# ayumiymk/DiG

Measured on AMD Instinct MI355X. Metric: pretrain images/sec (32x128, 2-view, mask 0.7) ViT-S/4, higher is better.
Workload: dtype bf16

## Files before the change

cpu_abi/dig_cpu.cpp:

```cpp
#include <algorithm>
#include <cmath>
#include <cstdint>
#include <cstring>
#include <vector>

typedef void* hipStream_t;
#include "../include/dig_block_types.h"
enum { DIG_OK = 0, DIG_ERR_ARG = -1, DIG_ERR_ALIGN = -2, DIG_ERR_LAUNCH = -3, DIG_ERR_UNSUPPORTED = -4 };
typedef uint16_t bf16_t;

struct dig_dropout_t {
  unsigned k0, k1, thr;
  float scale;
  unsigned pk0, pk1, pthr;
  float pscale;
  int rows_per_sample;
};

namespace {

inline float bf2f(bf16_t h) {
  const uint32_t u = (uint32_t)h << 16;
  float f;
  std::memcpy(&f, &u, 4);
// ... 1009 lines not shown
  for (int k = 0; k < 4; ++k) accs4[k] = stats6[(k >> 1) * 3 + 1 + (k & 1)] * acc_scale;
  return DIG_OK;
}
int dig_step_meters(const float* loss, const float* contra, const float* pixel, const float* accs4, const int* counts, int n_counts,
                    const float* grad_norm, float* out10, hipStream_t) {
  if (!loss || !contra || !pixel || !accs4 || !counts || n_counts <= 0 || !out10) return DIG_ERR_ARG;
  int lo = counts[0], hi = counts[0];
  for (int i = 1; i < n_counts; ++i) { lo = std::min(lo, counts[i]); hi = std::max(hi, counts[i]); }
  out10[0] = loss[0]; out10[1] = contra[0]; out10[2] = pixel[0];
  for (int k = 0; k < 4; ++k) out10[3 + k] = accs4[k];
  out10[7] = (float)lo; out10[8] = (float)hi; out10[9] = grad_norm ? grad_norm[0] : NAN;
  return DIG_OK;
}
int dig_ce_rows(float* logits, int n, int m, int label_offset, float gscale, float* out3, hipStream_t) {
  if (!logits || !out3 || n <= 0 || m <= 0 || label_offset < 0 || label_offset + n > m) return DIG_ERR_ARG;
  for (int i = 0; i < n; ++i) {
    float* row = logits + (size_t)i * m;
    const int label = i + label_offset;
    float mx = -3.0e38f;
    for (int j = 0; j < m; ++j) mx = std::max(mx, row[j]);
    const float zl = row[label];
    float s = 0.f;
    int gt = 0;
    for (int j = 0; j < m; ++j) { s += std::exp(row[j] - mx); gt += row[j] > zl; }
    const float lse = mx + std::log(s);
    for (int j = 0; j < m; ++j) row[j] = gscale * (std::exp(row[j] - mx) / s - (j == label ? 1.f : 0.f));
    out3[0] += lse - zl;
    if (gt < 1) out3[1] += 1.f;
    if (gt < 5) out3[2] += 1.f;
  }
  return DIG_OK;
}

static int adamw_core(float* p, const float* g, float* m, float* v, bf16_t* shadow, long long n, const unsigned char* group, float lr0,
                      float wd0, float lr1, float wd1, float beta1, float beta2, float eps, float inv_bc1, float inv_sqrt_bc2,
                      float grad_scale, const float* finite_gate) {
  if (finite_gate && !std::isfinite(finite_gate[0])) return DIG_OK;
#pragma omp parallel for
  for (long long i = 0; i < n; ++i) {
    const int grp = group[i >> 8] & 0x7f;
    if (grp == 2) {
      if (shadow) shadow[i] = f2bf(p[i]);
      continue;
    }
    const float lr = grp ? lr1 : lr0, wd = grp ? wd1 : wd0;
    const float gk = g[i] * grad_scale;
    float P = p[i] * (1.0f - lr * wd);
    const float M = m[i] * beta1 + gk * (1.0f - beta1);
    const float V = v[i] * beta2 + gk * gk * (1.0f - beta2);
    P -= (lr * inv_bc1) * (M / (std::sqrt(V) * inv_sqrt_bc2 + eps));
    p[i] = P; m[i] = M; v[i] = V;
    if (shadow) shadow[i] = f2bf(P);
  }
  return DIG_OK;
}

int dig_adamw_bias_corrections(float beta1, float beta2, int step, float* out2) {
  if (!out2 || step < 1) return DIG_ERR_ARG;
  out2[0] = (float)(1.0 / (1.0 - std::pow((double)beta1, (double)step)));
  out2[1] = (float)(1.0 / std::sqrt(1.0 - std::pow((double)beta2, (double)step)));
  return DIG_OK;
}

struct AdamTrMat { long long off, dst_off; int rows, cols, tile0, pad; };

int dig_adamw_step_tr(float* p, const float* g, float* m, float* v, void* bf16_shadow, long long n, const unsigned char* group_flags, float lr0,
// ... 557 lines not shown
```

dig_amd/build.py:

```python
import os
import subprocess
import sys
from concurrent.futures import ThreadPoolExecutor

HERE = os.path.dirname(os.path.abspath(__file__))
CSRC = os.path.join(HERE, "csrc")
LIBDIR = os.path.join(HERE, "lib")
LIB = os.path.join(LIBDIR, "libdig_hip.so")
FLAGS = ["--offload-arch=gfx950", "-O3", "-std=c++17", "-fPIC", "-munsafe-fp-atomics", "-ffp-contract=fast",
         "-Wno-unused-result"]
FLAGS.append("-fno-slp-vectorize")
EXTRA_FLAGS = {"keyview.hip": ["-ffp-contract=off"], "abiaug.hip": ["-ffp-contract=off"]}


def sources():
    return sorted(f for f in os.listdir(CSRC) if f.endswith(".hip"))


def source_hash() -> str:
    import hashlib
    h = hashlib.sha256()
    files = sorted(os.path.join(CSRC, f) for f in os.listdir(CSRC) if f.endswith((".hip", ".h", ".inc")))
    inc = os.path.join(os.path.dirname(HERE), "include")
    files += sorted(os.path.join(inc, f) for f in os.listdir(inc) if f.endswith(".h"))
# ... 25 lines not shown
    for s in sources():
        src = os.path.join(CSRC, s)
        obj = os.path.join(objdir, s[:-4] + ".o")
        if force or _stale(obj, [src] + headers):
            jobs.append((src, obj))

    def cc(job):
        src, obj = job
        cmd = [hipcc] + FLAGS + EXTRA_FLAGS.get(os.path.basename(src), []) + ["-I", os.path.join(os.path.dirname(HERE), "include"), "-c", src, "-o", obj]
        r = subprocess.run(cmd, capture_output=True, text=True)
        if r.returncode != 0:
            raise RuntimeError(f"hipcc failed for {src}:\n{r.stderr}")
        if verbose:
            print("[dig_amd.build] compiled", os.path.basename(src), flush=True)

    with ThreadPoolExecutor(max_workers=min(8, max(1, len(jobs)))) as ex:
        list(ex.map(cc, jobs))
    objs = [os.path.join(objdir, s[:-4] + ".o") for s in sources()]
    if force or jobs or _stale(LIB, objs):
        r = subprocess.run([hipcc, "--offload-arch=gfx950", "-shared", "-fPIC", "-o", LIB] + objs,
                           capture_output=True, text=True)
        if r.returncode != 0:
            raise RuntimeError("link failed:\n" + r.stderr)
        if verbose:
            print("[dig_amd.build] linked", LIB, flush=True)
    return LIB


HOT_KERNELS = ("mlp_chain_kernel<1, true, false>", "mlp_chain_kernel<2, true, false>", "mlp_chain_kernel<0, true, false>",
               "wgrad_wide_kernel<3, 7>", "attn_block_kernel<true, 2>", "attn_block_kernel<false, 2>", "attn_bwd_kernel<false, 3, false>", "attn_bwd_kernel<false, 3, true>",
               "gemm_wide_kernel<false, true, 0, 4, 3, 2, 2, false, 64, 2, false>", "gemm_pwide_kernel<4, false, false>",
               "keyview_sample_kernel", "keyview_stage_a_kernel", "keyview_stage_b_kernel",
               "abiaug_sample_kernel", "abiaug_warp_kernel", "abiaug_det_kernel", "abiaug_tail_kernel",
               "lexicon_search_kernel")
LLVM_BIN = os.environ.get("DIG_LLVM_BIN", "/opt/rocm/lib/llvm/bin")


def kernel_resources():
    import re
    import tempfile
    rows = []
    objdir = os.path.join(LIBDIR, "obj")
    with tempfile.TemporaryDirectory() as tmp:
        for o in sorted(f for f in os.listdir(objdir) if f.endswith(".o")):
            fat, dev = os.path.join(tmp, o + ".fat"), os.path.join(tmp, o + ".co")
            r = subprocess.run([os.path.join(LLVM_BIN, "llvm-objcopy"), f"--dump-section=.hip_fatbin={fat}", os.path.join(objdir, o)], capture_output=True, text=True)
            if r.returncode != 0 or not os.path.exists(fat):
                continue
            subprocess.run([os.path.join(LLVM_BIN, "clang-offload-bundler"), "--unbundle", "--type=o", f"--input={fat}",
                            "--targets=hipv4-amdgcn-amd-amdhsa--gfx950", f"--output={dev}"], check=True, capture_output=True)
            notes = subprocess.run([os.path.join(LLVM_BIN, "llvm-readelf"), "--notes", dev], check=True, capture_output=True, text=True).stdout
            for blk in notes.split("- .agpr_count")[1:]:
                f = {k: re.search(rf"\.{k}:\s+(\S+)", blk) for k in ("name", "private_segment_fixed_size", "vgpr_count", "sgpr_count")}
                if not all(f.values()):
                    continue
                mangled = f["name"].group(1)
                try:
                    dm = subprocess.run(["c++filt", mangled], capture_output=True, text=True).stdout.strip() or mangled
                except OSError:
                    dm = mangled
                short = re.sub(r"^void ", "", dm).replace("(anonymous namespace)::", "")
                rows.append({"name": short, "object": o, "scratch": int(f["private_segment_fixed_size"].group(1)),
                             "vgpr": int(f["vgpr_count"].group(1)), "sgpr": int(f["sgpr_count"].group(1)),
                             "hot": any(short.startswith(h) for h in HOT_KERNELS)})
    return rows


# ... 12 lines not shown
```

dig_amd/csrc/loss.hip:

```cpp
#include "common.h"

namespace {

__global__ void l2norm_fwd_kernel(const float* __restrict__ x, float* __restrict__ y, float* __restrict__ inv_norm, int n, int C,
                                  float eps) {
  const int r = blockIdx.x * (blockDim.x >> 6) + (threadIdx.x >> 6);
  const int lane = threadIdx.x & 63;
  if (r >= n) return;
  float s = 0.f;
  for (int c = lane; c < C; c += 64) { const float v = x[(size_t)r * C + c]; s += v * v; }
  s = wave_sum(s);
  const float inv = 1.0f / fmaxf(sqrtf(s), eps);
  for (int c = lane; c < C; c += 64) y[(size_t)r * C + c] = x[(size_t)r * C + c] * inv;
  if (lane == 0) inv_norm[r] = inv;
}

__global__ void l2norm_bwd_kernel(const float* __restrict__ dy, const float* __restrict__ y, const float* __restrict__ inv_norm,
                                  float* __restrict__ dx, int n, int C) {
  const int r = blockIdx.x * (blockDim.x >> 6) + (threadIdx.x >> 6);
  const int lane = threadIdx.x & 63;
  if (r >= n) return;
  float s = 0.f;
  for (int c = lane; c < C; c += 64) s += y[(size_t)r * C + c] * dy[(size_t)r * C + c];
  s = wave_sum(s);
// ... 79 lines not shown
      atomicAdd(out, lse - zl);
      if (gt < 0.5f) atomicAdd(out + 1, 1.f);
      if (gt < 4.5f) atomicAdd(out + 2, 1.f);
    }
    return;
  }
  __shared__ float red2[256];
  const float mine[3] = {lse - zl, gt < 0.5f ? 1.f : 0.f, gt < 4.5f ? 1.f : 0.f};
  float tot[3];
  if (dig_grid_sum_last<3>(ws, mine, tot, red2)) { out[0] += tot[0]; out[1] += tot[1]; out[2] += tot[2]; }
}

__global__ void infonce_finish_kernel(const float* __restrict__ stats6, float loss_scale, float acc_scale, float* __restrict__ contra,
                                      float* __restrict__ accs4) {
  if (threadIdx.x == 0) contra[0] = (stats6[0] + stats6[3]) * loss_scale;
  if (threadIdx.x < 4) accs4[threadIdx.x] = stats6[(threadIdx.x >> 1) * 3 + 1 + (threadIdx.x & 1)] * acc_scale;
}

__global__ __launch_bounds__(64) void step_meters_kernel(const float* __restrict__ loss, const float* __restrict__ contra, const float* __restrict__ pixel,
                                                        const float* __restrict__ accs4, const int* __restrict__ counts, int n_counts,
                                                        const float* __restrict__ grad_norm, float* __restrict__ out10) {
  int lo = 0x7fffffff, hi = -0x7fffffff - 1;
  for (int i = threadIdx.x; i < n_counts; i += 64) { const int c = counts[i]; lo = min(lo, c); hi = max(hi, c); }
#pragma unroll
  for (int o = 32; o > 0; o >>= 1) { lo = min(lo, __shfl_xor(lo, o, 64)); hi = max(hi, __shfl_xor(hi, o, 64)); }
  if (threadIdx.x == 0) {
    out10[0] = loss[0]; out10[1] = contra[0]; out10[2] = pixel[0];
    out10[7] = (float)lo; out10[8] = (float)hi;
    out10[9] = grad_norm ? grad_norm[0] : __builtin_nanf("");
  }
  if (threadIdx.x < 4) out10[3 + threadIdx.x] = accs4[threadIdx.x];
}

}

extern "C" int dig_infonce_finish(const float* stats6, float loss_scale, float acc_scale, float* contra, float* accs4, hipStream_t stream) {
  if (!stats6 || !contra || !accs4) return DIG_ERR_ARG;
  hipLaunchKernelGGL(infonce_finish_kernel, dim3(1), dim3(64), 0, stream, stats6, loss_scale, acc_scale, contra, accs4);
  return dig_check_launch();
}

extern "C" int dig_step_meters(const float* loss, const float* contra, const float* pixel, const float* accs4, const int* counts, int n_counts,
                               const float* grad_norm, float* out10, hipStream_t stream) {
  if (!loss || !contra || !pixel || !accs4 || !counts || n_counts <= 0 || !out10) return DIG_ERR_ARG;
  hipLaunchKernelGGL(step_meters_kernel, dim3(1), dim3(64), 0, stream, loss, contra, pixel, accs4, counts, n_counts, grad_norm, out10);
  return dig_check_launch();
}

extern "C" int dig_l2norm_fwd(const float* x, float* y, float* inv_norm, int n, int C, float eps, hipStream_t stream) {
  if (!x || !y || !inv_norm || n <= 0 || C <= 0) return DIG_ERR_ARG;
  hipLaunchKernelGGL(l2norm_fwd_kernel, dim3((n + 3) / 4), dim3(256), 0, stream, x, y, inv_norm, n, C, eps);
  return dig_check_launch();
}

extern "C" int dig_l2norm_bwd(const float* dy, const float* y, const float* inv_norm, float* dx, int n, int C, hipStream_t stream) {
  if (!dy || !y || !inv_norm || !dx || n <= 0 || C <= 0) return DIG_ERR_ARG;
  hipLaunchKernelGGL(l2norm_bwd_kernel, dim3((n + 3) / 4), dim3(256), 0, stream, dy, y, inv_norm, dx, n, C);
  return dig_check_launch();
}

extern "C" int dig_sgemm(const float* A, const float* B, float* C, int I, int J, int R, int lda, int ldb, int ldc, int trans_b,
                         float alpha, int r_splits, hipStream_t stream) {
  if (!A || !B || !C || I <= 0 || J <= 0 || R <= 0 || r_splits < 1) return DIG_ERR_ARG;
  const int per = ((R + r_splits - 1) / r_splits + 63) / 64 * 64;
  if ((R + per - 1) / per != r_splits) return DIG_ERR_ARG;
  dim3 grid((J + 31) / 32, (I + 31) / 32, r_splits);
  if (trans_b)
    hipLaunchKernelGGL(sgemm_kernel<true>, grid, dim3(256), 0, stream, A, B, C, I, J, R, lda, ldb, ldc, alpha, per);
  else
    hipLaunchKernelGGL(sgemm_kernel<false>, grid, dim3(256), 0, stream, A, B, C, I, J, R, lda, ldb, ldc, alpha, per);
  return dig_check_launch();
}

extern "C" int dig_ce_rows_ws(float* logits, int n, int m, int label_offset, float gscale, float* out3, float* workspace, hipStream_t stream) {
  if (!logits || !out3 || n <= 0 || m <= 0 || label_offset < 0 || label_offset + n > m) return DIG_ERR_ARG;
  hipLaunchKernelGGL(ce_rows_kernel, dim3(n), dim3(256), 0, stream, logits, n, m, label_offset, gscale, out3, workspace);
  return dig_check_launch();
}
extern "C" int dig_ce_rows(float* logits, int n, int m, int label_offset, float gscale, float* out3, hipStream_t stream) {
  return dig_ce_rows_ws(logits, n, m, label_offset, gscale, out3, nullptr, stream);
}
```

dig_amd/engine_core.py:

```python
import ctypes
import functools
import itertools
import os
import weakref
from typing import Optional, Tuple

import torch

from . import block_calls as BC
from . import encoder_blocks as EB
from . import ops
from .arena import enc_block_views
from .parallel import LOCAL, LocalComm, bn_backward, bn_forward

BF16, F32 = torch.bfloat16, torch.float32
FWD_MODE = os.environ.get("DIG_FWD_MODE", "flip")
CHAIN_BWD_EVERY = max(1, int(os.environ.get("DIG_CHAIN_BWD_EVERY", "1")))
CHAIN_BWD_PHASE = int(os.environ.get("DIG_CHAIN_BWD_PHASE", "0"))
BATCH_REDUCE = os.environ.get("DIG_BATCH_REDUCE", "0") == "1"
FUSED_QV_BIAS_SUMS = os.environ.get("DIG_FUSED_QV_BIAS", "1") != "0"
WGRAD_GROUPING = os.environ.get("DIG_WGRAD_GROUPING", "block")
WGRAD_INLINE = os.environ.get("DIG_WGRAD_INLINE", "1") == "1"
WGRAD_DEFER = os.environ.get("DIG_WGRAD_DEFER", "auto").strip().lower()
if WGRAD_DEFER not in ("auto", "0", "1"):
# ... 337 lines not shown
            enc_m, ks = momentum_branch()
            del enc_m
            main.wait_stream(hi_st)
        else:
            side.wait_stream(main)
            with torch.cuda.stream(side):
                enc_m, ks = momentum_branch(heads=not dist_mode)
            enc, self.saved_enc = self.encoder_forward(ew_on, images, aug, mask_u8, True, path=self.path_on)
            self.enc = enc
            if not dist_mode:
                qs = online_heads(enc)
                main.wait_stream(side)
                if side is not main:
                    ks.record_stream(main)
                del enc_m
            else:
                main.wait_stream(side)
                enc_m.record_stream(main)
                if pp:
                    (masked2, self.saved_pix), (masked_m, _) = self.mlp_forward_pair(enc[:B * N], "pix_projector", "online", True,
                                                                                      enc_m[:B * N], "pix_projector_m", "momentum", False)
                else:
                    masked2, self.saved_pix, masked_m = enc[:B * N], None, enc_m[:B * N]
                pooled, self.saved_pnet = extract(masked2, enc, "patch_extractor", "online", True)
                pooled_m, _ = extract(masked_m, enc_m, "momentum_patch_extractor", "momentum", False)
                (qs, self.saved_proj), (ks, _) = self.mlp_forward_pair(pooled, "encoder_projection_layer", "online", True,
                                                                        pooled_m, "momentum_projection_layer", "momentum", False)
                qs, self.saved_pred = self.mlp_forward(qs, "predictor", "online", True)
                del enc_m, masked_m, pooled_m
        _mark("forward: both encoders + heads joined", dev)
        M._flat["bn_count"] += 1
        n = B * M.n_patch
        dim = M.moco_dim
        qf = torch.empty((2 * n, dim), device=dev, dtype=F32)
        kf = torch.empty((2 * n, dim), device=dev, dtype=F32)
        ops.cast_bf16_to_f32(qs, qf)
        ops.cast_bf16_to_f32(ks, kf)
        qn, self.q_inv = ops.l2norm_fwd(qf)
        kn, _ = ops.l2norm_fwd(kf)
        self.qn = qn
        if dist_mode:
            kall = comm.all_gather_cat(kn.view(1, 2, n, dim))
            k1_all = kall[:, 0].reshape(comm.world * n, dim).contiguous()
            k2_all = kall[:, 1].reshape(comm.world * n, dim).contiguous()
        else:
            k1_all, k2_all = kn[:n], kn[n:]
        mk = comm.world * n
        stats = torch.zeros((2, 3), device=dev, dtype=F32)
        self.dqn = torch.empty((2 * n, dim), device=dev, dtype=F32)
        gs = 2.0 * M.T / n
        for half, kk in ((0, k2_all), (1, k1_all)):
            logits = torch.empty((n, mk), device=dev, dtype=F32)
            ops.sgemm(qn[half * n:(half + 1) * n], kk, logits, n, mk, dim, False, 1.0 / M.T)
            ops.ce_rows(logits, n * comm.rank, gs, stats[half])
            ops.sgemm(logits, kk, self.dqn[half * n:(half + 1) * n], n, dim, mk, True, 1.0 / M.T)
        contra, accs = ops.infonce_finish(stats, 2.0 * M.T / n, 100.0 / n)
        if not M.use_pixel_target:
            vis_out = torch.empty((0, 0, M.dec_classes), device=dev, dtype=F32)
            self.mim_views = 0
        elif vis_out is None:
            vis_out, _ = decoder()
        _mark("forward: InfoNCE + SimMIM decoder done", dev)
        return contra, accs, vis_out

    def _decoder_forward(self, mask_u8, images, mim_views):
        M = self.m
        B, N, dev = images.shape[0], M.N, images.device
        per = M._mask_count(mask_u8, B)
        Mrows = mim_views * B * per
        Mp = (Mrows + 63) // 64 * 64
        idx, cnt = ops.mask_to_index(mask_u8[:mim_views * B], per)
        M._last_mask_counts, M._last_idx, M._last_images = cnt, idx[:B], images
        M._last_idx_views = [idx[:B]] + ([(idx[B:] - B * N).clamp_min_(0)] if mim_views == 2 else [])
        self.idx, self.Mrows, self.Mp, self.per, self.mim_views = idx, Mrows, Mp, per, mim_views
        w16, f32 = M._w("online"), M._f32
        gath = ops.gather_rows(self.enc, idx, Mrows, Mp)
        h0 = ops.linear_fwd(gath, w16["pix_decoder.0.weight"])
        h1 = ops.linear_fwd(h0, w16["pix_decoder.1.weight"])
        h2, mu, rs = ops.layernorm_fwd(h1, f32["pix_decoder.2.weight"], f32["pix_decoder.2.bias"], M.ln_eps, gelu=True)
        pred = torch.empty((Mp, 64), device=dev, dtype=F32)
        C = M.dec_classes
        ops.gemm(h2, w16["pix_decoder.4.weight"], Mp, C, M.dec_dim, out=pred, out_kind=ops.OUT_F32, bias=f32["pix_decoder.4.bias"], ldc=64)
        self.saved_dec = (gath, h0, h1, h2, mu, rs)
        return pred[:Mrows, :C].reshape(mim_views * B, per, C)

    def _forward_gen_only(self, ew_on, images, aug, mask_u8, mim_views, training, fresh):
        M = self.m
        dev = images.device
        views = mim_views
        self.gen_views = views
        self.wT = None
        if training and ((ops.mlp_chain_supported(M.D, M.F, views * self.B * M.N) and (ops.MLP_CHAIN_MASK & 4)) or
                         (ops.DGRAD_DIRECT and views * self.B * M.N >= 8192)):
            self.wT = self.mlp_weight_transposes(ew_on, fresh)
        enc_raw, self.saved_enc = self.encoder_forward(ew_on, images, aug, mask_u8, True, views=views, path=self.path_on)
        f32 = M._f32
        self.enc, mu, rs = ops.layernorm_fwd(enc_raw, f32["encoder.norm.weight"], f32["encoder.norm.bias"], M.ln_eps)
        self.saved_norm = (enc_raw, mu, rs)
        vis_out = self._decoder_forward(mask_u8, images, mim_views)
        return torch.zeros((), device=dev, dtype=F32), torch.zeros(4, device=dev, dtype=F32), vis_out

    def backward(self, g_contra, g_vis):
        M = self.m
        B, D, N, nw = self.B, M.D, M.N, M.num_windows
        dev = self.enc.device
        w16, f32, g32 = M._w("online"), M._f32, M._g32
        contrast = g_contra is not None and M.use_moco_target
        if g_vis is not None and not M.use_pixel_target:
            g_vis = None
        self._assign, M._grads_fresh = bool(getattr(M, "_grads_fresh", False)), False
        _mark("backward: start (loss, MSE, autograd entry done)", dev)
        views = 2 if (contrast or (g_vis is not None and self.mim_views == 2)) else 1
        d_enc = torch.empty_like(self.enc) if contrast else torch.zeros((views * B * N, D), device=dev, dtype=BF16)
        n = B * M.n_patch
        if contrast:
            dqn = self.dqn
            ops.scale_by_device_scalar(dqn, g_contra.reshape(1).float())
            dq = ops.l2norm_bwd(dqn, self.qn, self.q_inv)
            dq16 = torch.empty(dq.shape, device=dev, dtype=BF16)
            ops.cast_f32_to_bf16(dq, dq16)
            dproj = self.mlp_backward(dq16, "predictor", self.saved_pred)
            self._grad_ready(dev, "predictor")
            dpool = self.mlp_backward(dproj, "encoder_projection_layer", self.saved_proj)
            self._grad_ready(dev, "encoder_projection_layer")
            acc = False
            if M.patchnet == 'regular':
                from . import patchnet
                dpool, dfeat = patchnet.backward(self, dpool, "patch_extractor", self.saved_pnet, 2 * B)
                self._grad_ready(dev, "patch_extractor")
                d_enc, acc = dfeat, True
            if M.patchnet == 'conv':
                from . import convpatchnet
                d_enc = convpatchnet.backward(self, dpool, "patch_extractor", self.saved_pnet, 2 * B)
                self._grad_ready(dev, "patch_extractor")
                if M.has_pix_projector:
                    self.mlp_backward(d_enc[:B * N], "pix_projector", self.saved_pix, dx_out=d_enc[:B * N])
                    self._grad_ready(dev, "pix_projector")
            elif M.has_pix_projector:
                dmasked2 = d_enc[:B * N] if acc else torch.empty((B * N, D), device=dev, dtype=BF16)
                ops.window_pool_bwd(dpool[:n], dmasked2, B, M.gh, M.gw, nw, D, acc)
                ops.window_pool_bwd(dpool[n:], d_enc[B * N:], B, M.gh, M.gw, nw, D, acc)
                self.mlp_backward(dmasked2, "pix_projector", self.saved_pix, dx_out=d_enc[:B * N])
                self._grad_ready(dev, "pix_projector")
            else:
                ops.window_pool_bwd(dpool[:n], d_enc[:B * N], B, M.gh, M.gw, nw, D, acc)
                ops.window_pool_bwd(dpool[n:], d_enc[B * N:], B, M.gh, M.gw, nw, D, acc)
        elif M.use_moco_target:
            for name in (("predictor", "encoder_projection_layer") + (("patch_extractor",) if M.patchnet != 'no_patchtrans' else ())
                         + (("pix_projector",) if M.has_pix_projector else ())):
                self.comm.grad_ready(M, name)
        if g_vis is not None:
            gath, h0, h1, h2, mu, rs = self.saved_dec
            Mrows, Mp, C, Dd = self.Mrows, self.Mp, M.dec_classes, M.dec_dim
# ... 133 lines not shown
```

dig_amd/ops.py:

```python
import ctypes
import os
from collections import namedtuple

import torch

from . import _lib as L

cf = ctypes.c_float
cll = ctypes.c_longlong
BF16 = torch.bfloat16
F32 = torch.float32

OUT_BF16, OUT_F32, OUT_F32_PARTIAL = 0, 1, 2
GEMM_BK_FWD, GEMM_BK_BWD = 64, 32
_ws = {}


def _stream_id(dev):
    if L._raw_stream is not None and dev.index is not None:
        return L._raw_stream(dev.index)
    return torch.cuda.current_stream(dev).cuda_stream


def _workspace(dev, numel):
# ... 829 lines not shown
    L.call("dig_bn_update_running", L.ptr(sums), cf(n_total), cf(momentum), L.ptr(rm), L.ptr(rv), rm.numel(), L.stream())


def bn_bwd_stats(dy, x, mean, rstd, gamma, beta, relu, sums, dbeta=None, dgamma=None):
    ws = _workspace2(x.device, _bn_ws_floats(x.shape[0], x.shape[1]))
    L.call("dig_bn_bwd_stats_acc", L.ptr(dy), L.ptr(x), L.ptr(mean), L.ptr(rstd), L.ptr(gamma), L.ptr(beta), int(relu), L.ptr(sums),
           L.ptr(dbeta), L.ptr(dgamma), L.ptr(ws), x.shape[0], x.shape[1], L.stream())


def bn_bwd_apply(dy, x, mean, rstd, gamma, beta, relu, sums, n_total):
    dx = torch.empty_like(x)
    L.call("dig_bn_bwd_apply", L.ptr(dy), L.ptr(x), L.ptr(mean), L.ptr(rstd), L.ptr(gamma), L.ptr(beta), int(relu), L.ptr(sums),
           cf(n_total), L.ptr(dx), x.shape[0], x.shape[1], L.stream())
    return dx


def l2norm_fwd(x, eps=1e-12):
    y = torch.empty_like(x)
    inv = torch.empty(x.shape[0], device=x.device, dtype=F32)
    L.call("dig_l2norm_fwd", L.ptr(x), L.ptr(y), L.ptr(inv), x.shape[0], x.shape[1], cf(eps), L.stream())
    return y, inv


def l2norm_bwd(dy, y, inv):
    dx = torch.empty_like(y)
    L.call("dig_l2norm_bwd", L.ptr(dy), L.ptr(y), L.ptr(inv), L.ptr(dx), y.shape[0], y.shape[1], L.stream())
    return dx


SGEMM_SPLIT_SMALL = os.environ.get("DIG_SGEMM_SPLIT_SMALL", "1") != "0"
SGEMM_SPLIT_MIN_R = 256


def sgemm(A, B, C, I, J, R, trans_b, alpha):
    sp = 1
    if R >= 2048 and C.stride(0) == J:
        sp = R // 512
        while sp > 1 and R % (64 * sp):
            sp -= 1
    elif SGEMM_SPLIT_SMALL and R >= SGEMM_SPLIT_MIN_R and I * J <= (1 << 18) and C.stride(0) == J and R % 256 == 0:
        sp = R // 128
    if sp > 1:
        ws = _workspace(A.device, sp * I * J)
        L.call("dig_sgemm", L.ptr(A), L.ptr(B), L.ptr(ws), I, J, R, A.stride(0), B.stride(0), J, int(trans_b), cf(alpha), sp, L.stream())
        L.call("dig_reduce_partials", L.ptr(ws), sp, cll(I * J), L.ptr(C), 0, L.stream())
    else:
        L.call("dig_sgemm", L.ptr(A), L.ptr(B), L.ptr(C), I, J, R, A.stride(0), B.stride(0), C.stride(0), int(trans_b), cf(alpha), 1, L.stream())


def ce_rows(logits, label_offset, gscale, out3):
    n = logits.shape[0]
    L.call("dig_ce_rows_ws", L.ptr(logits), n, logits.shape[1], label_offset, cf(gscale), L.ptr(out3),
           L.ptr(_loss_workspace(logits.device, "ce", 1 + 3 * n)), L.stream())


def infonce_finish(stats, loss_scale, acc_scale):
    contra = torch.empty((), device=stats.device, dtype=F32)
    accs = torch.empty(4, device=stats.device, dtype=F32)
    L.call("dig_infonce_finish", L.ptr(stats), cf(loss_scale), cf(acc_scale), L.ptr(contra), L.ptr(accs), L.stream())
    return contra, accs


def step_meters(loss, contra, pixel, accs4, counts, grad_norm):
    out = torch.empty(10, device=loss.device, dtype=F32)
    L.call("dig_step_meters", L.ptr(loss), L.ptr(contra), L.ptr(pixel), L.ptr(accs4), L.ptr(counts), counts.numel(), L.ptr(grad_norm), L.ptr(out),
           L.stream())
    return out


def cast_f32_to_bf16(x, y, n=None):
    L.call("dig_cast_f32_to_bf16", L.ptr(x), L.ptr(y), cll(x.numel() if n is None else n), L.stream())


def cast_bf16_to_f32(x, y, n=None):
    L.call("dig_cast_bf16_to_f32", L.ptr(x), L.ptr(y), cll(x.numel() if n is None else n), L.stream())


def fill_f32(x, value=0.0):
    L.call("dig_fill_f32", L.ptr(x), cll(x.numel()), cf(value), L.stream())


def scale_f32(x, s):
    L.call("dig_scale_f32", L.ptr(x), cll(x.numel()), cf(s), L.stream())


def scale_by_device_scalar(x, scalar, extra=1.0):
    L.call("dig_scale_by_device_scalar", L.ptr(x), cll(x.numel()), L.ptr(scalar), cf(extra), L.stream())


def pad_cast_rows(src, dst, M, C):
    L.call("dig_pad_cast_rows", L.ptr(src), L.ptr(dst), M, C, dst.shape[0], dst.stride(0), L.stream())


def axpy_f32(y, x, a=1.0):
    L.call("dig_axpy_f32", L.ptr(y), L.ptr(x), cll(x.numel()), cf(a), L.stream())
# ... 36 lines not shown
```

include/dig_hip.h:

```cpp
#ifndef DIG_HIP_H
#define DIG_HIP_H

#ifdef __cplusplus
extern "C" {
#endif

#ifndef __HIP_PLATFORM_AMD__
typedef struct ihipStream_t* hipStream_t;
#endif

#include "dig_aug_types.h"

#define DIG_GEMM_TILE_DEFAULT 0
#define DIG_GEMM_TILE_128x128_K32 32
#define DIG_GEMM_TILE_128x128_K64 64
#define DIG_GEMM_TILE_256x256 244
#define DIG_GEMM_TILE_256x192 264
#define DIG_GEMM_TILE_64x128 212
#define DIG_GEMM_TILE_128x64 221
#define DIG_GEMM_TILE_256x256_PERSISTENT 544
#define DIG_GEMM_TILE_256x192_PERSISTENT 564
int dig_gemm_bf16(const void* A, const void* B, void* C, int I, int J, int R, int lda, int ldb, int ldc, int trans_a,
                  int trans_b, int out_kind, const float* bias, const void* resid, int ldr, void* pre_act, int ldp, float alpha,
                  int alpha_cols, int act, int splits, int a_rows, int b_rows, int bk, float* colsum_partials,
// ... 92 lines not shown
int dig_patch_embed_bwd(const void* dy, const float* img, const unsigned char* mask, float* dW, float* dbias, float* dmask_token,
                        int n_img, int gh, int gw, int D, hipStream_t stream);
int dig_patchify_bf16(const float* img, const unsigned char* mask, void* out, int n_img, int gh, int gw, hipStream_t stream);
int dig_colsum_masked(const void* x, const unsigned char* mask, float* out_unmasked, float* out_masked, float* workspace,
                      int rows, int C, hipStream_t stream);

int dig_window_pool_fwd(const void* x, void* out, int out_is_f32, int n_img, int gh, int gw, int nwin, int D, hipStream_t stream);
int dig_window_pool_bwd(const void* dpool, void* dx, int n_img, int gh, int gw, int nwin, int D, int accumulate, hipStream_t stream);

int dig_im2col3x3(const void* x, void* col, int n_img, int H, int W, int C, int ldc, hipStream_t stream);
int dig_conv3x3_weight_flip(const void* w, void* wt, int c_out, int c_in, hipStream_t stream);
int dig_maxpool2x2_fwd(const void* x, void* y, unsigned char* idx, int n_img, int H, int W, int C, hipStream_t stream);
int dig_maxpool2x2_bwd(const void* dy, const unsigned char* idx, void* dx, int n_img, int H, int W, int C, hipStream_t stream);

int dig_mask_views_u8(const void* mask, int elem_kind, int B, int V, int N, int keep_views, unsigned char* out, hipStream_t stream);
int dig_mask_to_index(const unsigned char* mask, int* idx, int* count, int B, int N, int max_per_sample, hipStream_t stream);
int dig_gather_rows(const void* src, const int* idx, void* dst, int M, int M_pad, int D, hipStream_t stream);
int dig_scatter_rows_add(const void* src, const int* idx, void* dst, int M, int D, hipStream_t stream);
int dig_mim_target(const float* img, const int* idx, float* target, int M, int gh, int gw, int normalize , hipStream_t stream);
int dig_mse_fwd_bwd(const float* pred, int ld_pred, const float* target, int M, int C, float gscale, float* loss, void* dpred,
                    int ld_dpred, hipStream_t stream);

int dig_l2norm_fwd(const float* x, float* y, float* inv_norm, int n, int C, float eps, hipStream_t stream);
int dig_l2norm_bwd(const float* dy, const float* y, const float* inv_norm, float* dx, int n, int C, hipStream_t stream);
int dig_sgemm(const float* A, const float* B, float* C, int I, int J, int R, int lda, int ldb, int ldc, int trans_b, float alpha,
              int r_splits , hipStream_t stream);
int dig_ce_rows(float* logits, int n, int m, int label_offset, float gscale, float* out3, hipStream_t stream);
int dig_mse_fwd_bwd_ws(const float* pred, int ld_pred, const float* target, int M, int C, float gscale, float* loss, void* dpred,
                       int ld_dpred, float* workspace, hipStream_t stream);
int dig_ce_rows_ws(float* logits, int n, int m, int label_offset, float gscale, float* out3, float* workspace, hipStream_t stream);
int dig_infonce_finish(const float* stats6, float loss_scale, float acc_scale, float* contra, float* accs4, hipStream_t stream);
int dig_step_meters(const float* loss, const float* contra, const float* pixel, const float* accs4, const int* counts, int n_counts,
                    const float* grad_norm, float* out10, hipStream_t stream);

int dig_adamw_step(float* p, const float* g, float* m, float* v, void* bf16_shadow, long long n, const unsigned char* group_flags,
                   float lr0, float wd0, float lr1, float wd1, float beta1, float beta2, float eps, int step, float grad_scale,
                   const float* finite_gate, hipStream_t stream);
int dig_adamw_step_tr(float* p, const float* g, float* m, float* v, void* bf16_shadow, long long n, const unsigned char* group_flags,
                      float lr0, float wd0, float lr1, float wd1, float beta1, float beta2, float eps, int step, float grad_scale,
                      const float* finite_gate, const void* mats, int n_mats, int n_tiles, void* tr_out, hipStream_t stream);
int dig_adamw_step_groups(float* p, const float* g, float* m, float* v, void* bf16_shadow, long long n, const unsigned char* group_idx,
                          const float* lr_tab, const float* wd_tab, float beta1, float beta2, float eps, int step, float grad_scale,
                          const float* finite_gate, hipStream_t stream);
int dig_ema_update(float* pm, const float* p, void* bf16_shadow, long long n, float m, hipStream_t stream);
int dig_adamw_bias_corrections(float beta1, float beta2, int step, float* out2_host);
int dig_adamw_step_dev(float* p, const float* g, float* m, float* v, void* bf16_shadow, long long n, const unsigned char* group_flags,
                       const float* scalars6, float beta1, float beta2, float eps, float grad_scale, const float* finite_gate,
                       hipStream_t stream);
int dig_ema_update_dev(float* pm, const float* p, void* bf16_shadow, long long n, const float* m_and_one_minus_m, hipStream_t stream);
long long dig_sumsq_workspace_bytes(long long n);
int dig_sumsq(const float* x, long long n, float* workspace, float* out, hipStream_t stream);

long long dig_colsum_workspace_bytes(int rows, int C);
int dig_colsum(const void* x, float* out, float* workspace, int rows, int C, int ld, hipStream_t stream);
int dig_colsum_partials(const float* partials, int n_parts, int C, float* out, hipStream_t stream);
#define DIG_COLSUM_MAX_SEGS 112
typedef struct dig_colsum_seg { const float* partials; float* out; long long stride; int n_parts; int C; } dig_colsum_seg_t;
int dig_colsum_partials_multi(const dig_colsum_seg_t* segs, int n_segs, hipStream_t stream);
int dig_gelu_bwd(const void* dact, const void* pre, void* dpre, long long n, hipStream_t stream);
int dig_add_bf16(const void* a, const void* b, void* out, long long n, hipStream_t stream);
int dig_cast_f32_to_bf16(const float* x, void* y, long long n, hipStream_t stream);
int dig_cast_bf16_to_f32(const void* x, float* y, long long n, hipStream_t stream);
int dig_pad_cast_rows(const float* src, void* dst, int M, int C, int M_pad, int ld, hipStream_t stream);
int dig_fill_f32(float* x, long long n, float value, hipStream_t stream);
int dig_scale_f32(float* x, long long n, float s, hipStream_t stream);
int dig_scale_by_device_scalar(float* x, long long n, const float* scalar, float extra, hipStream_t stream);
// ... 129 lines not shown
```

Before: 6788.

## Fuse InfoNCE normalize, logits, softmax-CE and dq backward into dedicated kernels

Replaces the multi-launch InfoNCE path (bf16 casts, l2norm, two sgemms per direction, ce_rows, finish, scale, l2norm backward, cast) with three kernels. One normalizes the keys and writes a transposed copy, one computes per-block-of-8-query logits, softmax cross-entropy, gradient and dq with a last-block reduction of the stats, and one fuses scaling, l2norm backward and the bf16 cast. The aim is to cut launch count and intermediate global traffic while keeping the same split-K summation order as the sgemm path. In exchange the path handles only limited key counts and dims, uses 1024-thread blocks with low grid parallelism, and is bypassed in distributed mode.

```diff
diff --git a/cpu_abi/dig_cpu.cpp b/cpu_abi/dig_cpu.cpp
--- a/cpu_abi/dig_cpu.cpp
+++ b/cpu_abi/dig_cpu.cpp
@@ -1065,6 +1065,62 @@
   return DIG_OK;
 }
 
+int dig_infonce_keys(const void* k, float* kn, float* knT, int rows, int C, int rows_per_part, float eps, hipStream_t st) {
+  if (!k || !kn || !knT || rows <= 0 || C <= 0 || rows_per_part <= 0 || rows % rows_per_part) return DIG_ERR_ARG;
+  std::vector<float> x((size_t)rows * C), inv(rows);
+  const bf16_t* kb = (const bf16_t*)k;
+  for (size_t e = 0; e < x.size(); ++e) x[e] = bf2f(kb[e]);
+  dig_l2norm_fwd(x.data(), kn, inv.data(), rows, C, eps, st);
+  for (int r = 0; r < rows; ++r)
+    for (int c = 0; c < C; ++c)
+      knT[((size_t)(r / rows_per_part) * C + c) * rows_per_part + r % rows_per_part] = kn[(size_t)r * C + c];
+  return DIG_OK;
+}
+
+static void nce_sliced_gemm(const float* A, const float* B, float* C, int I, int J, int R, bool trans_b, float alpha, int per) {
+  for (int i = 0; i < I; ++i)
+    for (int j = 0; j < J; ++j) {
+      float tot = 0.f;
+      for (int r0 = 0; r0 < R; r0 += per) {
+        float acc = 0.f;
+        for (int r = r0; r < std::min(R, r0 + per); ++r) acc += A[(size_t)i * R + r] * (trans_b ? B[(size_t)r * J + j] : B[(size_t)j * R + r]);
+        tot += alpha * acc;
+      }
+      C[(size_t)i * J + j] = tot;
+    }
+}
+
+int dig_infonce_rows(const void* q, const float* kn_a, const float* knT_a, const float* kn_b, const float* knT_b, int n, int m, int C,
+                     int label_offset, float alpha, float gscale, float eps, int per_l, int per_d, float loss_scale, float acc_scale,
+                     float* qn, float* q_inv, float* dqn, float* contra, float* accs4, float* workspace, hipStream_t st) {
+  if (!q || !kn_a || !knT_a || !kn_b || !knT_b || !qn || !q_inv || !dqn || !contra || !accs4 || !workspace || n <= 0 || m <= 0 || C <= 0 ||
+      label_offset < 0 || label_offset + n > m || per_l <= 0 || per_d <= 0)
+    return DIG_ERR_ARG;
+  if (m > 1024 || C > 256 || ((C + per_l - 1) / per_l) * (long long)m > 2048 || ((m + per_d - 1) / per_d) * (long long)C > 2048) return DIG_ERR_UNSUPPORTED;
+  std::vector<float> x((size_t)2 * n * C), logits((size_t)n * m);
+  const bf16_t* qb = (const bf16_t*)q;
+  for (size_t e = 0; e < x.size(); ++e) x[e] = bf2f(qb[e]);
+  dig_l2norm_fwd(x.data(), qn, q_inv, 2 * n, C, eps, st);
+  float stats[6] = {0.f, 0.f, 0.f, 0.f, 0.f, 0.f};
+  for (int dir = 0; dir < 2; ++dir) {
+    const float* kn = dir ? kn_b : kn_a;
+    nce_sliced_gemm(qn + (size_t)dir * n * C, kn, logits.data(), n, m, C, false, alpha, per_l);
+    dig_ce_rows(logits.data(), n, m, label_offset, gscale, stats + 3 * dir, st);
+    nce_sliced_gemm(logits.data(), kn, dqn + (size_t)dir * n * C, n, C, m, true, alpha, per_d);
+  }
+  return dig_infonce_finish(stats, loss_scale, acc_scale, contra, accs4, st);
+}
+
+int dig_infonce_dq(const float* dqn, const float* qn, const float* q_inv, const float* gscalar, void* dq, int n, int C, hipStream_t st) {
+  if (!dqn || !qn || !q_inv || !gscalar || !dq || n <= 0 || C <= 0) return DIG_ERR_ARG;
+  std::vector<float> dy((size_t)n * C), dx((size_t)n * C);
+  for (size_t e = 0; e < dy.size(); ++e) dy[e] = dqn[e] * gscalar[0];
+  dig_l2norm_bwd(dy.data(), qn, q_inv, dx.data(), n, C, st);
+  bf16_t* o = (bf16_t*)dq;
+  for (size_t e = 0; e < dx.size(); ++e) o[e] = f2bf(dx[e]);
+  return DIG_OK;
+}
+
 static int adamw_core(float* p, const float* g, float* m, float* v, bf16_t* shadow, long long n, const unsigned char* group, float lr0,
                       float wd0, float lr1, float wd1, float beta1, float beta2, float eps, float inv_bc1, float inv_sqrt_bc2,
                       float grad_scale, const float* finite_gate) {
diff --git a/dig_amd/build.py b/dig_amd/build.py
--- a/dig_amd/build.py
+++ b/dig_amd/build.py
@@ -81,7 +81,8 @@
                "gemm_wide_kernel<false, true, 0, 4, 3, 2, 2, false, 64, 2, false>", "gemm_pwide_kernel<4, false, false>",
                "keyview_sample_kernel", "keyview_stage_a_kernel", "keyview_stage_b_kernel",
                "abiaug_sample_kernel", "abiaug_warp_kernel", "abiaug_det_kernel", "abiaug_tail_kernel",
-               "lexicon_search_kernel")
+               "lexicon_search_kernel",
+               "infonce_keys_kernel", "infonce_rows_kernel", "infonce_dq_kernel")
 LLVM_BIN = os.environ.get("DIG_LLVM_BIN", "/opt/rocm/lib/llvm/bin")
 
 
diff --git a/dig_amd/csrc/loss.hip b/dig_amd/csrc/loss.hip
--- a/dig_amd/csrc/loss.hip
+++ b/dig_amd/csrc/loss.hip
@@ -135,6 +135,253 @@
   if (threadIdx.x < 4) out10[3 + threadIdx.x] = accs4[threadIdx.x];
 }
 
+constexpr int NCE_RB = 8;
+constexpr int NCE_KG = 4;
+constexpr int NCE_CMAX = 256;
+
+__device__ __forceinline__ float nce_rounded(float v) {
+  asm volatile("" : "+v"(v));
+  return v;
+}
+
+__global__ void infonce_keys_kernel(const bf16_t* __restrict__ k, float* __restrict__ kn, float* __restrict__ knT, int rows, int C,
+                                    int rows_per_part, float eps) {
+  const int r = blockIdx.x * (blockDim.x >> 6) + (threadIdx.x >> 6);
+  const int lane = threadIdx.x & 63;
+  if (r >= rows) return;
+  float s = 0.f;
+  for (int c = lane; c < C; c += 64) { const float v = bf2f(k[(size_t)r * C + c]); s += v * v; }
+  s = wave_sum(s);
+  const float inv = 1.0f / fmaxf(sqrtf(s), eps);
+  const int part = r / rows_per_part, rp = r - part * rows_per_part;
+  float* t = knT + (size_t)part * C * rows_per_part + rp;
+  for (int c = lane; c < C; c += 64) {
+    const float y = bf2f(k[(size_t)r * C + c]) * inv;
+    kn[(size_t)r * C + c] = y;
+    t[(size_t)c * rows_per_part] = y;
+  }
+}
+
+__device__ __forceinline__ void nce_slice(const float* __restrict__ g, size_t ld, const float (*lds)[NCE_RB], int r0, int r1, float (&acc)[NCE_RB]) {
+#pragma unroll
+  for (int ii = 0; ii < NCE_RB; ++ii) acc[ii] = 0.f;
+  for (int r = r0; r < r1; r += 16) {
+    float kv[16];
+#pragma unroll
+    for (int e = 0; e < 16; ++e) kv[e] = g[(size_t)min(r + e, r1 - 1) * ld];
+#pragma unroll
+    for (int e = 0; e < 16; ++e)
+      if (r + e < r1) {
+        const float4 a = *reinterpret_cast<const float4*>(&lds[r + e][0]), b = *reinterpret_cast<const float4*>(&lds[r + e][4]);
+        acc[0] = fmaf(a.x, kv[e], acc[0]); acc[1] = fmaf(a.y, kv[e], acc[1]); acc[2] = fmaf(a.z, kv[e], acc[2]); acc[3] = fmaf(a.w, kv[e], acc[3]);
+        acc[4] = fmaf(b.x, kv[e], acc[4]); acc[5] = fmaf(b.y, kv[e], acc[5]); acc[6] = fmaf(b.z, kv[e], acc[6]); acc[7] = fmaf(b.w, kv[e], acc[7]);
+      }
+  }
+}
+
+__global__ __launch_bounds__(1024) void infonce_rows_kernel(const bf16_t* __restrict__ q, const float* __restrict__ kn_a,
+                                                            const float* __restrict__ knT_a, const float* __restrict__ kn_b,
+                                                            const float* __restrict__ knT_b, int n, int m, int C, int label_offset,
+                                                            float alpha, float gscale, float eps, int per_l, int per_d, float loss_scale,
+                                                            float acc_scale, float* __restrict__ qn, float* __restrict__ q_inv,
+                                                            float* __restrict__ dqn, float* __restrict__ contra, float* __restrict__ accs4,
+                                                            float* __restrict__ ws) {
+  __shared__ __attribute__((aligned(16))) float Qs[NCE_CMAX][NCE_RB];
+  __shared__ __attribute__((aligned(16))) float Dl[NCE_KG * 256][NCE_RB];
+  __shared__ float red[3][NCE_RB][4];
+  __shared__ unsigned last_flag;
+  const int nb = (n + NCE_RB - 1) / NCE_RB;
+  const int dir = blockIdx.x / nb, i0 = (blockIdx.x - dir * nb) * NCE_RB;
+  const float* __restrict__ kn = dir ? kn_b : kn_a;
+  const float* __restrict__ knT = dir ? knT_b : knT_a;
+  const int t = threadIdx.x, lane = t & 63, w = t >> 6;
+
+  if (w < NCE_RB) {
+    const int ii = w;
+    if (i0 + ii < n) {
+      const size_t g = (size_t)(dir * n + i0 + ii) * C;
+      float s = 0.f;
+      for (int c = lane; c < C; c += 64) { const float v = bf2f(q[g + c]); s += v * v; }
+      s = wave_sum(s);
+      const float inv = 1.0f / fmaxf(sqrtf(s), eps);
+      for (int c = lane; c < C; c += 64) {
+        const float y = bf2f(q[g + c]) * inv;
+        qn[g + c] = y;
+        Qs[c][ii] = y;
+      }
+      if (lane == 0) q_inv[dir * n + i0 + ii] = inv;
+    } else {
+      for (int c = lane; c < C; c += 64) Qs[c][ii] = 0.f;
+    }
+  }
+  __syncthreads();
+
+  {
+    const int nsl = (C + per_l - 1) / per_l, items = nsl * m;
+    float part[2][NCE_RB];
+#pragma unroll
+    for (int k = 0; k < 2; ++k) {
+      const int wi = t + 1024 * k;
+      if (wi < items) {
+        const int sl = wi / m, j = wi - sl * m;
+        nce_slice(knT + j, (size_t)m, Qs, sl * per_l, min(C, (sl + 1) * per_l), part[k]);
+      }
+    }
+    for (int sl = 0; sl < nsl; ++sl) {
+#pragma unroll
+      for (int k = 0; k < 2; ++k) {
+        const int wi = t + 1024 * k;
+        if (wi < items && wi / m == sl) {
+          const int j = wi - sl * m;
+#pragma unroll
+          for (int ii = 0; ii < NCE_RB; ++ii) Dl[j][ii] = (sl ? Dl[j][ii] : 0.f) + nce_rounded(part[k][ii] * alpha);
+        }
+      }
+      __syncthreads();
+    }
+  }
+
+  float lse[NCE_RB], zl[NCE_RB], gts[NCE_RB];
+  float lg[NCE_KG][NCE_RB], mx[NCE_RB];
+  if (t < 256) {
+#pragma unroll
+    for (int ii = 0; ii < NCE_RB; ++ii) {
+      float v = -3.0e38f;
+#pragma unroll
+      for (int u = 0; u < NCE_KG; ++u) {
+        lg[u][ii] = (t + 256 * u < m) ? Dl[t + 256 * u][ii] : 0.f;
+        if (t + 256 * u < m) v = fmaxf(v, lg[u][ii]);
+      }
+      v = wave_max(v);
+      if (lane == 0) red[0][ii][w] = v;
+      zl[ii] = Dl[min(i0 + ii + label_offset, m - 1)][ii];
+    }
+  }
+  __syncthreads();
+  if (t < 256) {
+#pragma unroll
+    for (int ii = 0; ii < NCE_RB; ++ii) {
+      mx[ii] = fmaxf(fmaxf(red[0][ii][0], red[0][ii][1]), fmaxf(red[0][ii][2], red[0][ii][3]));
+      float s = 0.f, gt = 0.f;
+#pragma unroll
+      for (int u = 0; u < NCE_KG; ++u)
+        if (t + 256 * u < m) {
+          const float z = lg[u][ii];
+          s += __expf(z - mx[ii]);
+          gt += (z > zl[ii]) ? 1.f : 0.f;
+        }
+      s = wave_sum(s);
+      gt = wave_sum(gt);
+      if (lane == 0) { red[1][ii][w] = s; red[2][ii][w] = gt; }
+    }
+  }
+  __syncthreads();
+  if (t < 256) {
+#pragma unroll
+    for (int ii = 0; ii < NCE_RB; ++ii) {
+      const float s = red[1][ii][0] + red[1][ii][1] + red[1][ii][2] + red[1][ii][3];
+      gts[ii] = red[2][ii][0] + red[2][ii][1] + red[2][ii][2] + red[2][ii][3];
+      lse[ii] = mx[ii] + __logf(s);
+      const float inv = 1.0f / s;
+      const int label = i0 + ii + label_offset;
+#pragma unroll
+      for (int u = 0; u < NCE_KG; ++u) {
+        const int j = t + 256 * u;
+        if (j < m) {
+          const float p = __expf(lg[u][ii] - mx[ii]) * inv;
+          Dl[j][ii] = gscale * (p - (j == label ? 1.f : 0.f));
+        }
+      }
+    }
+  }
+  __syncthreads();
+
+  {
+    const int nsl = (m + per_d - 1) / per_d, items = nsl * C;
+    float part[2][NCE_RB];
+#pragma unroll
+    for (int k = 0; k < 2; ++k) {
+      const int wi = t + 1024 * k;
+      if (wi < items) {
+        const int sl = wi / C, c = wi - sl * C;
+        nce_slice(kn + c, (size_t)C, Dl, sl * per_d, min(m, (sl + 1) * per_d), part[k]);
+      }
+    }
+    for (int sl = 0; sl < nsl; ++sl) {
+#pragma unroll
+      for (int k = 0; k < 2; ++k) {
+        const int wi = t + 1024 * k;
+        if (wi < items && wi / C == sl) {
+          const int c = wi - sl * C;
+#pragma unroll
+          for (int ii = 0; ii < NCE_RB; ++ii) Qs[c][ii] = (sl ? Qs[c][ii] : 0.f) + nce_rounded(part[k][ii] * alpha);
+        }
+      }
+      __syncthreads();
+    }
+    for (int e = t; e < NCE_RB * C; e += 1024) {
+      const int ii = e / C, c = e - ii * C;
+      if (i0 + ii < n) dqn[(size_t)(dir * n + i0 + ii) * C + c] = Qs[c][ii];
+    }
+  }
+
+  if (t == 0) {
+#pragma unroll
+    for (int ii = 0; ii < NCE_RB; ++ii)
+      if (i0 + ii < n) {
+        float* o = ws + 1 + 3 * (size_t)(dir * n + i0 + ii);
+        o[0] = lse[ii] - zl[ii]; o[1] = gts[ii] < 0.5f ? 1.f : 0.f; o[2] = gts[ii] < 4.5f ? 1.f : 0.f;
+      }
+    __threadfence();
+    last_flag = (atomicAdd(reinterpret_cast<unsigned*>(ws), 1u) == gridDim.x - 1) ? 1u : 0u;
+  }
+  __syncthreads();
+  if (!last_flag) return;
+  __threadfence();
+  float* fold = &Dl[0][0];
+  if (t < 256) {
+    float a[6];
+#pragma unroll
+    for (int v = 0; v < 6; ++v) a[v] = 0.f;
+    for (int b = t; b < n; b += 256) {
+#pragma unroll
+      for (int v = 0; v < 6; ++v)
+        a[v] += __hip_atomic_load(ws + 1 + 3 * (size_t)((v / 3) * n + b) + (v % 3), __ATOMIC_RELAXED, __HIP_MEMORY_SCOPE_AGENT);
+    }
+#pragma unroll
+    for (int v = 0; v < 6; ++v) {
+      a[v] = wave_sum(a[v]);
+      if (lane == 0) fold[w * 6 + v] = a[v];
+    }
+  }
+  __syncthreads();
+  if (t != 0) return;
+  float st[6];
+#pragma unroll
+  for (int v = 0; v < 6; ++v) {
+    float x = 0.f;
+    for (int ww = 0; ww < 4; ++ww) x += fold[ww * 6 + v];
+    st[v] = 0.f + x;
+  }
+  contra[0] = (st[0] + st[3]) * loss_scale;
+  accs4[0] = st[1] * acc_scale; accs4[1] = st[2] * acc_scale; accs4[2] = st[4] * acc_scale; accs4[3] = st[5] * acc_scale;
+  reinterpret_cast<unsigned*>(ws)[0] = 0u;
+}
+
+__global__ void infonce_dq_kernel(const float* __restrict__ dqn, const float* __restrict__ y, const float* __restrict__ inv_norm,
+                                  const float* __restrict__ gscalar, bf16_t* __restrict__ dq, int n, int C) {
+  const int r = blockIdx.x * (blockDim.x >> 6) + (threadIdx.x >> 6);
+  const int lane = threadIdx.x & 63;
+  if (r >= n) return;
+  const float sc = gscalar[0] * 1.0f;
+  float s = 0.f;
+  for (int c = lane; c < C; c += 64) s += y[(size_t)r * C + c] * nce_rounded(dqn[(size_t)r * C + c] * sc);
+  s = wave_sum(s);
+  const float inv = inv_norm[r];
+  for (int c = lane; c < C; c += 64)
+    dq[(size_t)r * C + c] = f2bf((nce_rounded(dqn[(size_t)r * C + c] * sc) - y[(size_t)r * C + c] * s) * inv);
+}
+
 }
 
 extern "C" int dig_infonce_finish(const float* stats6, float loss_scale, float acc_scale, float* contra, float* accs4, hipStream_t stream) {
@@ -183,3 +430,31 @@
 extern "C" int dig_ce_rows(float* logits, int n, int m, int label_offset, float gscale, float* out3, hipStream_t stream) {
   return dig_ce_rows_ws(logits, n, m, label_offset, gscale, out3, nullptr, stream);
 }
+
+extern "C" int dig_infonce_keys(const void* k, float* kn, float* knT, int rows, int C, int rows_per_part, float eps, hipStream_t stream) {
+  if (!k || !kn || !knT || rows <= 0 || C <= 0 || rows_per_part <= 0 || rows % rows_per_part) return DIG_ERR_ARG;
+  hipLaunchKernelGGL(infonce_keys_kernel, dim3((rows + 3) / 4), dim3(256), 0, stream, (const bf16_t*)k, kn, knT, rows, C, rows_per_part, eps);
+  return dig_check_launch();
+}
+
+extern "C" int dig_infonce_rows(const void* q, const float* kn_a, const float* knT_a, const float* kn_b, const float* knT_b, int n, int m, int C,
+                                int label_offset, float alpha, float gscale, float eps, int per_l, int per_d, float loss_scale,
+                                float acc_scale, float* qn, float* q_inv, float* dqn, float* contra, float* accs4, float* workspace,
+                                hipStream_t stream) {
+  if (!q || !kn_a || !knT_a || !kn_b || !knT_b || !qn || !q_inv || !dqn || !contra || !accs4 || !workspace || n <= 0 || m <= 0 || C <= 0 ||
+      label_offset < 0 || label_offset + n > m || per_l <= 0 || per_d <= 0)
+    return DIG_ERR_ARG;
+  if (m > NCE_KG * 256 || C > NCE_CMAX || ((C + per_l - 1) / per_l) * (long long)m > 2048 || ((m + per_d - 1) / per_d) * (long long)C > 2048)
+    return DIG_ERR_UNSUPPORTED;
+  hipLaunchKernelGGL(infonce_rows_kernel, dim3(2 * ((n + NCE_RB - 1) / NCE_RB)), dim3(1024), 0, stream, (const bf16_t*)q, kn_a, knT_a, kn_b,
+                     knT_b, n, m, C, label_offset, alpha, gscale, eps, per_l, per_d, loss_scale, acc_scale, qn, q_inv, dqn, contra, accs4,
+                     workspace);
+  return dig_check_launch();
+}
+
+extern "C" int dig_infonce_dq(const float* dqn, const float* qn, const float* q_inv, const float* gscalar, void* dq, int n, int C,
+                              hipStream_t stream) {
+  if (!dqn || !qn || !q_inv || !gscalar || !dq || n <= 0 || C <= 0) return DIG_ERR_ARG;
+  hipLaunchKernelGGL(infonce_dq_kernel, dim3((n + 3) / 4), dim3(256), 0, stream, dqn, qn, q_inv, gscalar, (bf16_t*)dq, n, C);
+  return dig_check_launch();
+}
diff --git a/dig_amd/engine_core.py b/dig_amd/engine_core.py
--- a/dig_amd/engine_core.py
+++ b/dig_amd/engine_core.py
@@ -393,6 +393,11 @@
         M._flat["bn_count"] += 1
         n = B * M.n_patch
         dim = M.moco_dim
+        self.nce_fused = ops.INFONCE_FUSED and not dist_mode and ops.infonce_fused_supported(n, n, dim)
+        if self.nce_fused:
+            kn, knT = ops.infonce_keys(ks, 2)
+            contra, accs, self.qn, self.q_inv, self.dqn = ops.infonce_rows(qs, (kn[n:], knT[1]), (kn[:n], knT[0]), M.T)
+            return self._infonce_tail(contra, accs, vis_out, decoder, dev)
         qf = torch.empty((2 * n, dim), device=dev, dtype=F32)
         kf = torch.empty((2 * n, dim), device=dev, dtype=F32)
         ops.cast_bf16_to_f32(qs, qf)
@@ -416,6 +421,10 @@
             ops.ce_rows(logits, n * comm.rank, gs, stats[half])
             ops.sgemm(logits, kk, self.dqn[half * n:(half + 1) * n], n, dim, mk, True, 1.0 / M.T)
         contra, accs = ops.infonce_finish(stats, 2.0 * M.T / n, 100.0 / n)
+        return self._infonce_tail(contra, accs, vis_out, decoder, dev)
+
+    def _infonce_tail(self, contra, accs, vis_out, decoder, dev):
+        M = self.m
         if not M.use_pixel_target:
             vis_out = torch.empty((0, 0, M.dec_classes), device=dev, dtype=F32)
             self.mim_views = 0
@@ -476,10 +485,13 @@
         n = B * M.n_patch
         if contrast:
             dqn = self.dqn
-            ops.scale_by_device_scalar(dqn, g_contra.reshape(1).float())
-            dq = ops.l2norm_bwd(dqn, self.qn, self.q_inv)
-            dq16 = torch.empty(dq.shape, device=dev, dtype=BF16)
-            ops.cast_f32_to_bf16(dq, dq16)
+            if self.nce_fused:
+                dq16 = ops.infonce_dq(dqn, self.qn, self.q_inv, g_contra.reshape(1).float())
+            else:
+                ops.scale_by_device_scalar(dqn, g_contra.reshape(1).float())
+                dq = ops.l2norm_bwd(dqn, self.qn, self.q_inv)
+                dq16 = torch.empty(dq.shape, device=dev, dtype=BF16)
+                ops.cast_f32_to_bf16(dq, dq16)
             dproj = self.mlp_backward(dq16, "predictor", self.saved_pred)
             self._grad_ready(dev, "predictor")
             dpool = self.mlp_backward(dproj, "encoder_projection_layer", self.saved_proj)
diff --git a/dig_amd/ops.py b/dig_amd/ops.py
--- a/dig_amd/ops.py
+++ b/dig_amd/ops.py
@@ -885,14 +885,23 @@
 SGEMM_SPLIT_MIN_R = 256
 
 
-def sgemm(A, B, C, I, J, R, trans_b, alpha):
+def sgemm_splits(I, J, R, dense=True):
     sp = 1
-    if R >= 2048 and C.stride(0) == J:
+    if R >= 2048 and dense:
         sp = R // 512
         while sp > 1 and R % (64 * sp):
             sp -= 1
-    elif SGEMM_SPLIT_SMALL and R >= SGEMM_SPLIT_MIN_R and I * J <= (1 << 18) and C.stride(0) == J and R % 256 == 0:
+    elif SGEMM_SPLIT_SMALL and R >= SGEMM_SPLIT_MIN_R and I * J <= (1 << 18) and dense and R % 256 == 0:
         sp = R // 128
+    return sp
+
+
+def sgemm_slice_len(R, sp):
+    return ((R + sp - 1) // sp + 63) // 64 * 64
+
+
+def sgemm(A, B, C, I, J, R, trans_b, alpha):
+    sp = sgemm_splits(I, J, R, C.stride(0) == J)
     if sp > 1:
         ws = _workspace(A.device, sp * I * J)
         L.call("dig_sgemm", L.ptr(A), L.ptr(B), L.ptr(ws), I, J, R, A.stride(0), B.stride(0), J, int(trans_b), cf(alpha), sp, L.stream())
@@ -914,6 +923,44 @@
     return contra, accs
 
 
+INFONCE_FUSED = os.environ.get("DIG_INFONCE_FUSED", "1") != "0"
+INFONCE_MAX_KEYS, INFONCE_MAX_DIM = 1024, 256
+
+
+def infonce_fused_supported(n, m, dim):
+    if m > INFONCE_MAX_KEYS or dim > INFONCE_MAX_DIM:
+        return False
+    return sgemm_splits(n, m, dim) * m <= 2048 and sgemm_splits(n, dim, m) * dim <= 2048
+
+
+def infonce_keys(ks, parts, eps=1e-12):
+    rows, dim = ks.shape
+    kn = torch.empty((rows, dim), device=ks.device, dtype=F32)
+    knT = torch.empty((parts, dim, rows // parts), device=ks.device, dtype=F32)
+    L.call("dig_infonce_keys", L.ptr(ks), L.ptr(kn), L.ptr(knT), rows, dim, rows // parts, cf(eps), L.stream())
+    return kn, knT
+
+
+def infonce_rows(qs, keys_a, keys_b, T, label_offset=0, eps=1e-12):
+    dim, dev = qs.shape[1], qs.device
+    n, m = qs.shape[0] // 2, keys_a[0].shape[0]
+    qn, dqn = torch.empty((2 * n, dim), device=dev, dtype=F32), torch.empty((2 * n, dim), device=dev, dtype=F32)
+    q_inv = torch.empty(2 * n, device=dev, dtype=F32)
+    contra, accs = torch.empty((), device=dev, dtype=F32), torch.empty(4, device=dev, dtype=F32)
+    per_l = sgemm_slice_len(dim, sgemm_splits(n, m, dim))
+    per_d = sgemm_slice_len(m, sgemm_splits(n, dim, m))
+    L.call("dig_infonce_rows", L.ptr(qs), L.ptr(keys_a[0]), L.ptr(keys_a[1]), L.ptr(keys_b[0]), L.ptr(keys_b[1]), n, m, dim, label_offset,
+           cf(1.0 / T), cf(2.0 * T / n), cf(eps), per_l, per_d, cf(2.0 * T / n), cf(100.0 / n), L.ptr(qn), L.ptr(q_inv), L.ptr(dqn),
+           L.ptr(contra), L.ptr(accs), L.ptr(_loss_workspace(dev, "infonce", 1 + 6 * n)), L.stream())
+    return contra, accs, qn, q_inv, dqn
+
+
+def infonce_dq(dqn, qn, q_inv, gscalar):
+    dq = torch.empty(qn.shape, device=qn.device, dtype=BF16)
+    L.call("dig_infonce_dq", L.ptr(dqn), L.ptr(qn), L.ptr(q_inv), L.ptr(gscalar), L.ptr(dq), qn.shape[0], qn.shape[1], L.stream())
+    return dq
+
+
 def step_meters(loss, contra, pixel, accs4, counts, grad_norm):
     out = torch.empty(10, device=loss.device, dtype=F32)
     L.call("dig_step_meters", L.ptr(loss), L.ptr(contra), L.ptr(pixel), L.ptr(accs4), L.ptr(counts), counts.numel(), L.ptr(grad_norm), L.ptr(out),
diff --git a/include/dig_hip.h b/include/dig_hip.h
--- a/include/dig_hip.h
+++ b/include/dig_hip.h
@@ -148,6 +148,11 @@
 int dig_infonce_finish(const float* stats6, float loss_scale, float acc_scale, float* contra, float* accs4, hipStream_t stream);
 int dig_step_meters(const float* loss, const float* contra, const float* pixel, const float* accs4, const int* counts, int n_counts,
                     const float* grad_norm, float* out10, hipStream_t stream);
+int dig_infonce_keys(const void* k, float* kn, float* knT, int rows, int C, int rows_per_part, float eps, hipStream_t stream);
+int dig_infonce_rows(const void* q, const float* kn_a, const float* knT_a, const float* kn_b, const float* knT_b, int n, int m, int C,
+                     int label_offset, float alpha, float gscale, float eps, int per_l, int per_d, float loss_scale, float acc_scale,
+                     float* qn, float* q_inv, float* dqn, float* contra, float* accs4, float* workspace, hipStream_t stream);
+int dig_infonce_dq(const float* dqn, const float* qn, const float* q_inv, const float* gscalar, void* dq, int n, int C, hipStream_t stream);
 
 int dig_adamw_step(float* p, const float* g, float* m, float* v, void* bf16_shadow, long long n, const unsigned char* group_flags,
                    float lr0, float wd0, float lr1, float wd1, float beta1, float beta2, float eps, int step, float grad_scale,
```

After: 6834, median of 6. Within noise of the previous version (+0.7%).
